# NVIDIA/tacotron2

Measured on AMD Instinct MI355X. Metric: mel-frames/sec (train fwd+bwd) LJSpeech hparams, higher is better.
Workload: dtype bf16; 1 GPU; BASELINE configs[1]: LJSpeech default hparams, batch_size=64/GPU, synthetic LJSpeech-shaped batches, full train step (fwd+loss+bwd+clip+Adam); global_batch=64, parallelism=dp1, optimizer=FusedAdam, compute=bf16 MFMA operands, f32 accumulate/state/master weights

## Files before the change

include/tacotron2_amd.h:

```cpp
#ifndef TACOTRON2_AMD_H
#define TACOTRON2_AMD_H

#include <stdint.h>

#ifdef __cplusplus
extern "C" {
#endif

#define T2AMD_ABI_VERSION 1
#define T2AMD_OK 0
#define T2AMD_ERR_ARG 1
#define T2AMD_ERR_LAUNCH 2

#define T2AMD_ATT_DIM 128
#define T2AMD_LOC_FILTERS 32
#define T2AMD_LOC_KERNEL 31
#define T2AMD_LOC_TAPS (2 * T2AMD_LOC_KERNEL)
#define T2AMD_ATT_SLICES 4

int t2amd_abi_version(void);
const char* t2amd_source_sha1(void);
const char* t2amd_last_error(void);
int t2amd_struct_sizes(int* out, int max_n);
int t2amd_set_validate_only(int on);
// ... 31 lines not shown
                            long long n, int accumulate, int perm_taps, int perm_ci, void* stream);
int t2amd_splitk_reduce2d_f32(const float* partials, int nsplit, long long stride, float* out, int rows, int cols,
                              long long ldo, int accumulate, void* stream);

typedef struct t2amd_gemm16_desc {
    const void* A;
    const void* B;
    float* C;
    int M, N, K;
    long long lda, ldb, ldc;
    int splitk;
    long long strideSplitC;
    int accumulate;
    const float* bias;
    int win_T, win_Tp;
} t2amd_gemm16_desc;
int t2amd_gemm16_tn(const t2amd_gemm16_desc* d, void* stream);
int t2amd_gemm16_kk(const t2amd_gemm16_desc* d, void* stream);
int t2amd_gemm16_kk_group(const t2amd_gemm16_desc* d, int count, void* stream);

int t2amd_cast_halo_bf16(const float* src, long long lds, void* dst, long long rows, int C, int T, int pad, void* stream);

int t2amd_pack_conv_bf16(const float* W, void* out, int Co, int Ci, int k, int Kp, int reversed, void* stream);

int t2amd_transpose_cast_bf16(const void* src, int src_is_bf16, long long lds, void* dst, long long ldd, int rows, int cols,
                              int rows_padded, void* stream);

int t2amd_bn_stats_f32(const float* x, long long ldx, int M, int N, double* ws, float* mean,
                       float* invstd, float* running_mean, float* running_var, float momentum,
                       float eps, void* stream);
int t2amd_bn_eval_invstd_f32(const float* running_var, float* invstd, int N, float eps, void* stream);
// ... 564 lines not shown
```

tacotron2_amd/csrc/gemm16.hip:

```cpp
#include "common.h"
#include <stdlib.h>

typedef __bf16 g16_bf16x8 __attribute__((ext_vector_type(8)));
typedef __attribute__((address_space(3))) void* g16_lptr;
typedef __attribute__((address_space(1))) const void* g16_gptr;

#define G16_T 256
#define G16_BK 64
#define G16_IMG (G16_T * 128)
#define G16_NT 512

struct Gemm16Params {
    t2amd_gemm16_desc d;
    int ktiles_per_split;
};

struct G16Tile { int bx, by, bz; };
__device__ __forceinline__ G16Tile g16_tile_id() {
    const int nbx = gridDim.x, nby = gridDim.y;
    const int total = nbx * nby * (int)gridDim.z;
    const int L = blockIdx.x + nbx * (blockIdx.y + nby * blockIdx.z);
    const int xcd = L & 7, q = L >> 3;
    const int base = total >> 3, rem = total & 7;
    const int id = xcd * base + (xcd < rem ? xcd : rem) + q;
    const int per_z = nbx * nby;
    G16Tile t;
    t.bz = id / per_z;
    const int r = id - t.bz * per_z;
    const int G = 8;
    const int group = r / (G * nbx);
    const int first = group * G;
    const int gsz = (nby - first) < G ? (nby - first) : G;
    const int w = r - group * (G * nbx);
    t.by = first + w % gsz;
    t.bx = w / gsz;
    return t;
}

__global__ __launch_bounds__(G16_NT) void gemm16_tn_kernel(Gemm16Params p) {
    __shared__ __attribute__((aligned(16))) char smem[4 * G16_IMG];
    const t2amd_gemm16_desc& d = p.d;
    const int tid = threadIdx.x, lane = tid & 63;
    const int wave = __builtin_amdgcn_readfirstlane(tid >> 6);
    const int wm = wave >> 2, wn = wave & 3;
    const int l31 = lane & 31, lhi = lane >> 5;

    const G16Tile tile = g16_tile_id();
    const int split = tile.bz;
    const int row0 = tile.by * G16_T, col0 = tile.bx * G16_T;
    const int M = d.M, N = d.N;
    const int nkt_all = d.K / G16_BK;
    const int kt_beg = split * p.ktiles_per_split;
    int kt_end = kt_beg + p.ktiles_per_split;
// ... 91 lines not shown
            asm volatile("s_waitcnt vmcnt(0)" ::: "memory");
            __builtin_amdgcn_s_barrier();
            if (kt + 2 < nk) G16_ISSUE(0)
            G16_TILE(1)
            asm volatile("s_waitcnt vmcnt(0)" ::: "memory");
            __builtin_amdgcn_s_barrier();
        }
        if (nk & 1) G16_TILE(0)
    }
#undef G16_ISSUE
#undef G16_READ
#undef G16_WAIT
#undef G16_MFMA
#undef G16_TILE

    float* __restrict__ C = d.C + (long long)split * d.strideSplitC;
#pragma unroll
    for (int tm = 0; tm < 4; ++tm) {
#pragma unroll
        for (int tn = 0; tn < 2; ++tn) {
            const int gn = col0 + wn * 64 + tn * 32 + l31;
#pragma unroll
            for (int r = 0; r < 16; ++r) {
                const int gm = row0 + wm * 128 + tm * 32 + (r & 3) + 8 * (r >> 2) + 4 * lhi;
                long long crow = gm;
                bool live = gm < M;
                if (d.win_Tp > 0) {
                    const int b_ = gm / d.win_Tp, t_ = gm - b_ * d.win_Tp;
                    live = live && t_ < d.win_T;
                    crow = (long long)b_ * d.win_T + t_;
                }
                if (live && gn < N) {
                    float* cp = C + crow * d.ldc + gn;
                    float val = acc[tm][tn][r];
                    if (d.bias) val += d.bias[gn];
                    if (d.accumulate) val += *cp;
                    *cp = val;
                }
            }
        }
    }
}

extern "C" int t2amd_gemm16_tn(const t2amd_gemm16_desc* dp, void* stream) {
    T2_REQUIRE(dp != nullptr, "gemm16: null descriptor");
    Gemm16Params p;
    p.d = *dp;
    t2amd_gemm16_desc& d = p.d;
    T2_REQUIRE(d.A && d.B && d.C, "gemm16: null operand");
    T2_REQUIRE(d.M > 0 && d.N > 0 && d.K > 0 && d.K % G16_BK == 0, "gemm16: K must be a positive multiple of 64");
    T2_REQUIRE(t2_aligned16(d.A) && t2_aligned16(d.B) && d.lda % 8 == 0 && d.ldb % 8 == 0 && d.ldb >= d.K,
               "gemm16: operands must be 16-byte aligned with row strides that are multiples of 8 elements (B's >= K)");
    T2_REQUIRE(d.win_Tp == 0 || (d.win_T > 0 && d.win_T <= d.win_Tp && d.splitk == 1), "gemm16: bad window geometry");
    T2_REQUIRE(d.win_Tp > 0 || d.lda >= d.K, "gemm16: lda must be >= K unless the rows are windows");
    if (d.splitk < 1) d.splitk = 1;
    T2_REQUIRE(d.splitk == 1 || (!d.bias && !d.accumulate), "gemm16: split-K needs a plain epilogue");
    const int nkt = d.K / G16_BK;
    p.ktiles_per_split = t2_cdiv(nkt, d.splitk);
    dim3 grid(t2_cdiv(d.N, G16_T), t2_cdiv(d.M, G16_T), d.splitk);
    T2_REQUIRE(grid.y <= 65535 && grid.z <= 65535, "gemm16: grid too large");
    T2_LAUNCH(gemm16_tn_kernel, grid, dim3(G16_NT), 0, (hipStream_t)stream, p);
    T2_LAUNCH_CHECK();
    return T2AMD_OK;
}

typedef float g16_f32x2 __attribute__((ext_vector_type(2)));

#define G16_GROUP 4
struct Gemm16GroupParams {
    t2amd_gemm16_desc d[G16_GROUP];
    int coltile_end[G16_GROUP];
    int count;
};

__global__ __launch_bounds__(G16_NT) void gemm16_kk_kernel(Gemm16GroupParams p) {
    __shared__ __attribute__((aligned(16))) char smem[4 * G16_IMG];
    const int tid = threadIdx.x, lane = tid & 63;
    const int wave = __builtin_amdgcn_readfirstlane(tid >> 6);
    const int wm = wave >> 2, wn = wave & 3;
    const int l31 = lane & 31, lhi = lane >> 5;

    const G16Tile tile = g16_tile_id();
    const int split = tile.bz;
    int prob = 0;
#pragma unroll
    for (int j = 0; j + 1 < G16_GROUP; ++j)
        if (j + 1 < p.count && tile.bx >= p.coltile_end[j]) prob = j + 1;
    const int bx = tile.bx - (prob > 0 ? p.coltile_end[prob - 1] : 0);
    struct { const void* A; const void* B; float* C; int M, N, K; long long lda, ldb, ldc; long long strideSplitC; int accumulate;
// ... 127 lines not shown
            KK_LANDED(1, kt + 1)
            if (kt + 2 < nk) KK_ISSUE(0, kt + 2)
            KK_TILE(1)
            KK_LANDED(0, kt + 2)
        }
        if (nk & 1) KK_TILE(0)
    }
#undef KK_ISSUE
#undef KK_LANDED
#undef KK_READ
#undef KK_WAIT
#undef KK_OP
#undef KK_MFMA
#undef KK_TILE

    float* __restrict__ C = d.C + (long long)split * d.strideSplitC;
#pragma unroll
    for (int tm = 0; tm < 4; ++tm) {
#pragma unroll
        for (int tn = 0; tn < 2; ++tn) {
            const int gn = col0 + wn * 64 + tn * 32 + l31;
#pragma unroll
            for (int r = 0; r < 16; ++r) {
                const int gm = row0 + wm * 128 + tm * 32 + (r & 3) + 8 * (r >> 2) + 4 * lhi;
                if (gm < M && gn < N) {
                    float* cp = C + (long long)gm * d.ldc + gn;
                    float val = acc[tm][tn][r];
                    if (d.bias) val += d.bias[gn];
                    if (d.accumulate) val += *cp;
                    *cp = val;
// ... 6 lines not shown
extern "C" int t2amd_gemm16_kk_group(const t2amd_gemm16_desc* dp, int count, void* stream) {
    T2_REQUIRE(dp != nullptr && count >= 1 && count <= G16_GROUP, "gemm16_kk: 1..4 descriptors");
    Gemm16GroupParams p;
    p.count = count;
    int coltiles = 0;
    for (int j = 0; j < G16_GROUP; ++j) {
        p.d[j] = dp[j < count ? j : count - 1];
        if (j >= count) { p.coltile_end[j] = coltiles; continue; }
        t2amd_gemm16_desc& d = p.d[j];
        T2_REQUIRE(d.A && d.B && d.C, "gemm16_kk: null operand");
        T2_REQUIRE(d.M >= 8 && d.N >= 8 && d.K > 0 && d.M % 8 == 0 && d.N % 8 == 0, "gemm16_kk: M and N must be positive multiples of 8, K positive");
        T2_REQUIRE(t2_aligned16(d.A) && t2_aligned16(d.B) && d.lda > 0 && d.ldb > 0 && d.lda % 8 == 0 && d.ldb % 8 == 0,
                   "gemm16_kk: operands must be 16-byte aligned with row strides that are multiples of 8 elements");
        T2_REQUIRE(d.win_Tp == 0 && d.win_T == 0, "gemm16_kk: no window epilogue (overlapping rows are expressed by lda / ldb < M / N)");
        if (d.splitk < 1) d.splitk = 1;
        T2_REQUIRE(d.splitk == 1 || (!d.bias && !d.accumulate), "gemm16_kk: split-K needs a plain epilogue");
        T2_REQUIRE(d.M == p.d[0].M && d.splitk == p.d[0].splitk, "gemm16_kk: the products of one launch share M and the split count");
        coltiles += t2_cdiv(d.N, G16_T);
        p.coltile_end[j] = coltiles;
    }
    dim3 grid(coltiles, t2_cdiv(p.d[0].M, G16_T), p.d[0].splitk);
    T2_REQUIRE(grid.y <= 65535 && grid.z <= 65535, "gemm16_kk: grid too large");
    T2_LAUNCH(gemm16_kk_kernel, grid, dim3(G16_NT), 0, (hipStream_t)stream, p);
    T2_LAUNCH_CHECK();
    return T2AMD_OK;
}

extern "C" int t2amd_gemm16_kk(const t2amd_gemm16_desc* dp, void* stream) { return t2amd_gemm16_kk_group(dp, 1, stream); }

template <bool SRC16>
__global__ __launch_bounds__(256) void transpose_cast16_kernel(const void* __restrict__ src, long long lds_, unsigned short* __restrict__ dst,
                                                               long long ldd, int rows, int cols, int rpad) {
    __shared__ unsigned short tile[64][66];
    const int r0 = blockIdx.x * 64, c0 = blockIdx.y * 64;
    const int tid = threadIdx.x;
    const bool vec_in = SRC16 ? (lds_ % 4 == 0 && (reinterpret_cast<size_t>(src) & 7) == 0) : (lds_ % 4 == 0 && (reinterpret_cast<size_t>(src) & 15) == 0);
#pragma unroll
    for (int pass = 0; pass < 4; ++pass) {
        const int i = pass * 16 + (tid >> 4), j = 4 * (tid & 15);
// ... 113 lines not shown
```

tacotron2_amd/engine.py:

```python
import os

import math
import torch

from . import native as nv
from .native import NativeError

BN_EPS = 1e-5
BN_MOMENTUM = 0.1


def check_hparams(hp):
    if hp.n_frames_per_step != 1:
        raise ValueError("n_frames_per_step != 1 is not supported (nor by the reference, hparams.py:56)")
    K = hp.attention_location_kernel_size
    if not (1 <= hp.attention_dim <= nv.ATT_DIM and 1 <= hp.attention_location_n_filters <= nv.LOC_FILTERS
            and 1 <= K <= nv.LOC_KERNEL and K % 2 == 1):
        raise ValueError("the attention kernels hold attention_dim <= %d, <= %d location filters and an odd location "
                         "kernel <= %d (smaller geometries run zero-embedded in the compiled one; an even kernel size "
                         "does not run in the reference either: ConvNorm pads (k-1)//2, model.py:18-20)"
                         % (nv.ATT_DIM, nv.LOC_FILTERS, nv.LOC_KERNEL))
    for name in ('encoder_embedding_dim', 'attention_rnn_dim', 'decoder_rnn_dim', 'prenet_dim'):
        if getattr(hp, name) % 64 != 0:
            raise ValueError("%s must be a multiple of 64 for the MFMA recurrent kernels" % name)
# ... 73 lines not shown
            best, best_t = s, t
    return best


WGRAD16 = os.environ.get('T2AMD_WGRAD16', '1') != '0'


WGRAD_KK = os.environ.get('T2AMD_WGRAD_KK', '1') != '0'


def _kk_to(run, out, A16, B16, K, M, N, lda=None, ldb=None, perm=None):
    sk = _choose_splitk16(M, N, K)
    if sk == 1 and perm is None:
        nv.gemm16_kk(out, A16, B16, K, M=M, N=N, lda=lda, ldb=ldb)
        return
    part = run.empty(sk, M * N)
    nv.gemm16_kk(part[0].view(M, N), A16, B16, K, M=M, N=N, lda=lda, ldb=ldb, splitk=sk, partials=part)
    if perm is not None:
        nv.splitk_reduce(part, sk, out, perm_taps=perm[0], perm_ci=perm[1])
    else:
        nv.splitk_reduce2d(part, sk, out)


def _lstm_wgrad_kk(run, dG2, B, parts, outs):
    rowsD, G4 = dG2.shape
    widths = [src.shape[1] for src, _ in parts]
    offs = [0]
    for w in widths:
        offs.append(offs[-1] + w)
    jobs = []
    for dW, i0, i1 in outs:
        base = offs[i0]
        for i in range(i0, i1):
            src, shifted = parts[i]
            if src.dtype != torch.bfloat16:
                src = run.cast16(src)
            blk = dW[:, offs[i] - base:offs[i + 1] - base]
            if shifted and rowsD <= B:
                blk.zero_()
            elif shifted:
                jobs.append((blk, dG2[B:], src, rowsD - B, widths[i]))
            else:
                jobs.append((blk, dG2, src, rowsD, widths[i]))
    if not jobs:
        return
    sk = _choose_splitk16(G4, sum((j[4] + 255) // 256 * 256 for j in jobs), rowsD)
    if sk == 1:
        nv.gemm16_kk_group([dict(Cm=blk, A16=A, B16=Bm, K=K, M=G4, N=w) for blk, A, Bm, K, w in jobs])
        return
    parts_ = [run.empty(sk, G4 * w) for _, _, _, _, w in jobs]
    nv.gemm16_kk_group([dict(Cm=pt[0].view(G4, w), A16=A, B16=Bm, K=K, M=G4, N=w, splitk=sk, partials=pt)
                        for (blk, A, Bm, K, w), pt in zip(jobs, parts_)])
    for (blk, _, _, _, _), pt in zip(jobs, parts_):
        nv.splitk_reduce2d(pt, sk, blk)


def _lstm_wgrad16(run, dG2, B, parts, outs):
    rowsD, G4 = dG2.shape
    if WGRAD_KK and G4 % 8 == 0 and all(src.shape[1] % 8 == 0 for src, _ in parts):
        return _lstm_wgrad_kk(run, dG2, B, parts, outs)
    Kp = ((rowsD + B + 63) // 64) * 64
    GT = run.empty16(G4, Kp)
    nv.transpose_cast_bf16(dG2, GT)
    widths = [src.shape[1] for src, _ in parts]
    XT = run.empty16(sum(widths), Kp)
    n0, offs = 0, []
    for (src, shifted), w in zip(parts, widths):
        blk = XT[n0:n0 + w]
        if shifted:
# ... 2 lines not shown
                nv.transpose_cast_bf16(src[:rowsD - B], blk[:, B:])
            else:
                blk[:, B:].zero_()
        else:
            nv.transpose_cast_bf16(src, blk)
        offs.append(n0)
        n0 += w
    offs.append(n0)
    for dW, i0, i1 in outs:
        Bop = XT[offs[i0]:offs[i1]]
        M, N = dW.shape
        sk = _choose_splitk16(M, N, Kp)
        if sk == 1:
            nv.gemm16_tn(dW, GT, Bop)
        else:
            part = run.empty(sk, M * N)
            nv.gemm16_tn(dW, GT, Bop, splitk=sk, partials=part)
            nv.splitk_reduce(part, sk, dW)


class _Ctx(object):
    arena = None

    def release(self):
        a, self.arena = self.arena, None
        _arena_release(a)

    def __del__(self):
        try:
            self.release()
        except Exception:
            pass

# ... 1701 lines not shown
```

tacotron2_amd/native.py:

```python
import ctypes as C
import os

import torch

_HERE = os.path.dirname(os.path.abspath(__file__))
LIB_PATH = os.environ.get("T2AMD_LIB", os.path.join(_HERE, "lib", "libtacotron2_amd.so"))

TORCH_OPS_PATH = os.path.join(_HERE, "lib", "libtacotron2_amd_torch.so")

ATT_DIM = 128
LOC_FILTERS = 32
LOC_KERNEL = 31
LOC_TAPS = 62
ATT_SLICES = 4

_f32p = C.c_void_p
_i64 = C.c_longlong


class GemmDesc(C.Structure):
    _fields_ = [
        ("A", _f32p), ("B", _f32p), ("C", _f32p),
        ("M", C.c_int), ("N", C.c_int), ("K", C.c_int),
        ("lda", _i64), ("ldb", _i64), ("ldc", _i64),
# ... 5 lines not shown
        ("bias", _f32p), ("act", C.c_int),
        ("keep", C.c_void_p), ("ldkeep", _i64), ("keep_scale", C.c_float),
        ("convA_T", C.c_int), ("convA_C", C.c_int), ("convA_pad", C.c_int), ("convA_sign", C.c_int),
        ("convB_T", C.c_int), ("convB_C", C.c_int), ("convB_pad", C.c_int),
        ("precision", C.c_int),
    ]


class Gemm16Desc(C.Structure):
    _fields_ = [
        ("A", C.c_void_p), ("B", C.c_void_p), ("C", _f32p),
        ("M", C.c_int), ("N", C.c_int), ("K", C.c_int),
        ("lda", _i64), ("ldb", _i64), ("ldc", _i64),
        ("splitk", C.c_int), ("strideSplitC", _i64), ("accumulate", C.c_int), ("bias", _f32p),
        ("win_T", C.c_int), ("win_Tp", C.c_int),
    ]


class Seg(C.Structure):
    _fields_ = [("p", _f32p), ("ld", _i64), ("width", C.c_int)]


class LstmStep(C.Structure):
    _fields_ = [
        ("x", Seg * 3), ("nseg", C.c_int),
        ("W", _f32p), ("Ktot", C.c_int), ("H", C.c_int), ("B", C.c_int),
        ("gin", _f32p), ("ld_gin", _i64),
        ("bias", _f32p),
        ("c_prev", _f32p), ("ld_cprev", _i64),
        ("gates_out", _f32p), ("ld_gates", _i64),
# ... 178 lines not shown
    _fields_ = [("param", C.c_void_p * MAX_TENSORS), ("grad", C.c_void_p * MAX_TENSORS),
                ("exp_avg", C.c_void_p * MAX_TENSORS), ("exp_avg_sq", C.c_void_p * MAX_TENSORS),
                ("numel", C.c_longlong * MAX_TENSORS), ("first_block", C.c_int * MAX_TENSORS), ("count", C.c_int)]


class AdamHyper(C.Structure):
    _fields_ = [("step_size", C.c_float), ("bc2_sqrt", C.c_float), ("one_minus_beta1", C.c_float),
                ("beta2", C.c_float), ("one_minus_beta2", C.c_float), ("eps", C.c_float), ("weight_decay", C.c_float)]


_STRUCTS = [GemmDesc, Seg, LstmStep, SkinnyGemm, Addend, LstmBwd, AttnFwd, AttnBwd, DecTrain,
            DecTrainBwd, LstmSeq, DecInfer, SmallLinear, TensorList, AdamHyper, DecPersist, Gemm16Desc]

SYMBOLS = [
    "t2amd_abi_version", "t2amd_source_sha1", "t2amd_last_error", "t2amd_struct_sizes", "t2amd_set_validate_only", "t2amd_profile_enable", "t2amd_profile_read", "t2amd_profile_event_overhead",
    "t2amd_gemm_f32", "t2amd_gemm_tile_size", "t2amd_splitk_reduce_f32", "t2amd_splitk_reduce2d_f32", "t2amd_gemm16_tn", "t2amd_gemm16_kk", "t2amd_gemm16_kk_group", "t2amd_transpose_cast_bf16", "t2amd_cast_halo_bf16", "t2amd_pack_conv_bf16",
    "t2amd_bn_stats_f32", "t2amd_bn_eval_invstd_f32", "t2amd_bn_act_fwd_f32", "t2amd_bn_act_bwd_f32", "t2amd_bn_act_bwd_img_f32", "t2amd_colsum_bf16", "t2amd_bn_act_fwd_img_f32",
    "t2amd_colsum_f32",
    "t2amd_embedding_fwd_f32", "t2amd_embedding_bwd_f32", "t2amd_philox_keep_mask", "t2amd_fill_f32",
    "t2amd_copy2d_f32", "t2amd_cast_bf16_f32", "t2amd_split_bf16x3_f32", "t2amd_transpose_f32", "t2amd_frames_to_time_major_f32",
    "t2amd_split_projection_f32", "t2amd_finalize_outputs_f32", "t2amd_grads_to_channel_last_f32",
    "t2amd_gather_dout_f32", "t2amd_relu_dropout_bwd_f32",
    "t2amd_lstm_step_fwd_f32", "t2amd_skinny_gemm_f32", "t2amd_lstm_pointwise_bwd_f32",
    "t2amd_lstm_step_fwd2_f32", "t2amd_skinny_gemm2_f32", "t2amd_lstm_pointwise_bwd2_f32",
    "t2amd_fold_location_f32", "t2amd_unfold_location_grads_f32",
    "t2amd_attention_step_fwd_f32", "t2amd_attention_step_bwd_f32",
    "t2amd_decoder_train_fwd_loop_f32", "t2amd_decoder_train_bwd_loop_f32",
    "t2amd_decoder_train_fwd_persistent_flag_bytes", "t2amd_decoder_train_fwd_persistent_supported", "t2amd_decoder_train_fwd_persistent_f32",
    "t2amd_lstm_seq_fwd_f32", "t2amd_lstm_seq_bwd_f32", "t2amd_decoder_infer_steps_f32",
    "t2amd_set_decoder_streams", "t2amd_set_bptt_cell_fold", "t2amd_get_bptt_cell_fold", "t2amd_attn_bwd_ws_floats",
    "t2amd_set_small_batch_max", "t2amd_get_small_batch_max", "t2amd_dec_infer_uses_tiles",
# ... 16 lines not shown
]

_P, _I, _L, _F, _UL = C.c_void_p, C.c_int, C.c_longlong, C.c_float, C.c_ulonglong


def _argtypes():
    pt = C.POINTER
    return {
        "t2amd_gemm_f32": [pt(GemmDesc), _P],
        "t2amd_gemm_tile_size": [_I, _I, _I, _I, _I, _I],
        "t2amd_splitk_reduce_f32": [_P, _I, _L, _P, _L, _I, _I, _I, _P],
        "t2amd_splitk_reduce2d_f32": [_P, _I, _L, _P, _I, _I, _L, _I, _P],
        "t2amd_gemm16_tn": [pt(Gemm16Desc), _P],
        "t2amd_gemm16_kk": [pt(Gemm16Desc), _P],
        "t2amd_gemm16_kk_group": [pt(Gemm16Desc), _I, _P],
        "t2amd_transpose_cast_bf16": [_P, _I, _L, _P, _L, _I, _I, _I, _P],
        "t2amd_cast_halo_bf16": [_P, _L, _P, _L, _I, _I, _I, _P],
        "t2amd_pack_conv_bf16": [_P, _P, _I, _I, _I, _I, _I, _P],
        "t2amd_bn_stats_f32": [_P, _L, _I, _I, _P, _P, _P, _P, _P, _F, _F, _P],
        "t2amd_bn_eval_invstd_f32": [_P, _P, _I, _F, _P],
        "t2amd_bn_act_fwd_f32": [_P, _L, _P, _L, _I, _I, _P, _P, _P, _P, _I, _P, _L, _F, _P, _I, _P],
        "t2amd_bn_act_fwd_img_f32": [_P, _L, _P, _L, _I, _I, _P, _P, _P, _P, _I, _P, _L, _F, _P, _I, _I, _P],
        "t2amd_bn_act_bwd_f32": [_P, _L, _P, _L, _P, _L, _I, _I, _P, _P, _P, _I, _P, _L, _F, _P, _P, _P, _P],
        "t2amd_bn_act_bwd_img_f32": [_P, _L, _P, _L, _P, _L, _I, _I, _P, _P, _P, _I, _P, _L, _F, _P, _P, _P, _P, _I, _I, _P, _I, _P],
        "t2amd_colsum_f32": [_P, _L, _I, _I, _P, _P, _I, _P],
        "t2amd_colsum_bf16": [_P, _L, _I, _I, _P, _P, _I, _P],
        "t2amd_embedding_fwd_f32": [_P, _P, _P, _L, _I, _I, _P],
        "t2amd_embedding_bwd_f32": [_P, _P, _P, _P, _L, _I, _I, _P],
        "t2amd_philox_keep_mask": [_P, _L, _F, _UL, _UL, _P],
        "t2amd_fill_f32": [_P, _L, _F, _P],
# ... 118 lines not shown
    lib = C.CDLL(LIB_PATH)
    for name in SYMBOLS:
        if not hasattr(lib, name):
            raise NativeError("tacotron2_amd: symbol %s missing from %s" % (name, LIB_PATH))
    for name, at in _argtypes().items():
        fn = getattr(lib, name)
        fn.argtypes = at
        fn.restype = C.c_int
    lib.t2amd_last_error.restype = C.c_char_p
    lib.t2amd_reflect_index.argtypes = [_L, _L]
    lib.t2amd_reflect_index.restype = C.c_longlong
    lib.t2amd_gl_packed_rows.argtypes = [_P, _I, _I, _I]
    lib.t2amd_gl_packed_rows.restype = C.c_longlong
    lib.t2amd_abi_version.restype = C.c_int
    lib.t2amd_attn_bwd_ws_floats.restype = C.c_longlong
    lib.t2amd_attn_fwd_ws_floats.restype = C.c_longlong
    lib.t2amd_decoder_persist_mailbox_bytes.restype = C.c_longlong
    lib.t2amd_lstm_seq_persistent_mailbox_bytes.restype = C.c_longlong
    lib.t2amd_lstm_seq_batch_persistent_flag_bytes.restype = C.c_longlong
    lib.t2amd_decoder_train_fwd_persistent_flag_bytes.restype = C.c_longlong
    if lib.t2amd_abi_version() != 1:
        raise NativeError("tacotron2_amd: ABI version mismatch")
    lib.t2amd_source_sha1.restype = C.c_char_p
    lib.t2amd_source_sha1.argtypes = []
    built = (lib.t2amd_source_sha1() or b"").decode()
    if os.path.isdir(os.path.join(_HERE, "csrc")) and os.environ.get("T2AMD_ALLOW_STALE_LIB", "0") != "1":
        from . import build as _build
        try:
            want = _build.source_sha1()
        except OSError as e:
# ... 232 lines not shown
            raise NativeError("gemm: keep mask must be a [M,N] uint8 view, got %s" % (tuple(keep.shape),))
        d.keep, d.ldkeep, d.keep_scale = ptr(keep, torch.uint8), keep.stride(0), keep_scale
    if convA is not None:
        d.convA_T, d.convA_C, d.convA_pad, d.convA_sign = convA
    if convB is not None:
        d.convB_T, d.convB_C, d.convB_pad = convB
    if splitk > 1:
        if partials is None or partials.numel() < splitk * M * N or not partials.is_contiguous():
            raise NativeError("gemm: split-K needs a contiguous partials buffer")
        d.C = ptr(partials)
        d.ldc = N
        d.strideSplitC = M * N
    _check(lib.t2amd_gemm_f32(C.byref(d), _stream()), "t2amd_gemm_f32")


def gemm16_tn(Cm, A16, B16, K=None, splitk=1, partials=None, accumulate=False, bias=None):
    lib = load()
    d = Gemm16Desc()
    pa, lda, M, Ka = _mat(A16, torch.bfloat16)
    pb, ldb, N, Kb = _mat(B16, torch.bfloat16)
    K = Ka if K is None else K
    if K > Ka or K > Kb or Cm.shape[0] != M or Cm.shape[1] != N:
        raise NativeError("gemm16_tn: shape mismatch A=%s B=%s C=%s K=%d" % (tuple(A16.shape), tuple(B16.shape), tuple(Cm.shape), K))
    d.A, d.B, d.M, d.N, d.K, d.lda, d.ldb = pa, pb, M, N, K, lda, ldb
    d.splitk = splitk
    if splitk > 1:
        if partials is None or partials.numel() < splitk * M * N:
            raise NativeError("gemm16_tn: split-K needs a (splitk, M*N) partials buffer")
        d.C, d.ldc, d.strideSplitC = ptr(partials), N, M * N
    else:
        d.C, d.ldc = _mat(Cm)[:2]
    d.accumulate = 1 if accumulate else 0
    d.bias = ptr(bias)
    _check(lib.t2amd_gemm16_tn(C.byref(d), _stream()), "t2amd_gemm16_tn")


def conv16(Cm, img16, W16, B, T, pad, bias=None, accumulate=False):
    lib = load()
    d = Gemm16Desc()
    Ci = img16.shape[1]
    Tp = T + 2 * pad
    pw, ldw, Co, K = _mat(W16, torch.bfloat16)
    klen = (2 * pad + 1) * Ci
    if img16.shape[0] < B * Tp + 2 * pad or K < klen or K - klen > 2 * pad * Ci or Cm.shape[0] != B * T or Cm.shape[1] != Co:
        raise NativeError("conv16: shape mismatch img=%s W=%s C=%s" % (tuple(img16.shape), tuple(W16.shape), tuple(Cm.shape)))
    d.A, d.lda = ptr(_fullc(img16), torch.bfloat16), Ci
    d.B, d.ldb = pw, ldw
    d.C, d.ldc = _mat(Cm)[:2]
    d.M, d.N, d.K = (B - 1) * Tp + T, Co, K
    d.splitk, d.accumulate, d.bias = 1, 1 if accumulate else 0, ptr(bias)
    d.win_T, d.win_Tp = T, Tp
    _check(lib.t2amd_gemm16_tn(C.byref(d), _stream()), "t2amd_gemm16_tn")


def _kk_desc(Cm, A16, B16, K, M=None, N=None, lda=None, ldb=None, splitk=1, partials=None, accumulate=False, bias=None):
    d = Gemm16Desc()
    pa, lda0, ra, wa = _mat(A16, torch.bfloat16)
    pb, ldb0, rb, wb = _mat(B16, torch.bfloat16)
    M = wa if M is None else M
    N = wb if N is None else N
    lda = lda0 if lda is None else lda
    ldb = ldb0 if ldb is None else ldb
    span_a = (ra - 1) * lda0 + wa
    span_b = (rb - 1) * ldb0 + wb
    if K < 1 or (K - 1) * lda + M > span_a or (K - 1) * ldb + N > span_b or Cm.shape[0] != M or Cm.shape[1] != N:
        raise NativeError("gemm16_kk: shape mismatch A=%s B=%s C=%s M=%d N=%d K=%d lda=%d ldb=%d"
                          % (tuple(A16.shape), tuple(B16.shape), tuple(Cm.shape), M, N, K, lda, ldb))
    d.A, d.B, d.M, d.N, d.K, d.lda, d.ldb = pa, pb, M, N, K, lda, ldb
    d.splitk = splitk
    if splitk > 1:
        if partials is None or partials.numel() < splitk * M * N:
            raise NativeError("gemm16_kk: split-K needs a (splitk, M*N) partials buffer")
        d.C, d.ldc, d.strideSplitC = ptr(partials), N, M * N
    else:
        d.C, d.ldc = _mat(Cm)[:2]
    d.accumulate = 1 if accumulate else 0
    d.bias = ptr(bias)
    return d


def gemm16_kk(Cm, A16, B16, K, M=None, N=None, lda=None, ldb=None, splitk=1, partials=None, accumulate=False, bias=None):
    d = _kk_desc(Cm, A16, B16, K, M, N, lda, ldb, splitk, partials, accumulate, bias)
    _check(load().t2amd_gemm16_kk(C.byref(d), _stream()), "t2amd_gemm16_kk")


def gemm16_kk_group(problems):
    if not 1 <= len(problems) <= 4:
        raise NativeError("gemm16_kk_group: 1..4 problems, got %d" % len(problems))
    arr = (Gemm16Desc * len(problems))(*[_kk_desc(**kw) for kw in problems])
    reads = [kw[k_] for kw in problems for k_ in ('A16', 'B16')]
    writes = [kw['partials'] if kw.get('partials') is not None else kw['Cm'] for kw in problems]
    if not _via_ops("wgrad_gemm16", [arr], reads, writes):
        _check(load().t2amd_gemm16_kk_group(arr, len(problems), _stream()), "t2amd_gemm16_kk_group")


def pack_conv_bf16(W, reversed=False):
    Co, Ci, k = W.shape
    rows, inner = (Ci, Co) if reversed else (Co, Ci)
    Kp = (k * inner + 63) // 64 * 64
    out = torch.empty(rows, Kp, dtype=torch.bfloat16, device=W.device)
    _check(load().t2amd_pack_conv_bf16(ptr(_fullc(W)), ptr(out, torch.bfloat16), Co, Ci, k, Kp, 1 if reversed else 0, _stream()),
           "t2amd_pack_conv_bf16")
    return out


def cast_halo_bf16(src, dst, T, pad):
# ... 1187 lines not shown
```

Measured before the change: 648,400 valid mel-frames/s.

## Fuse split-K reduction into gemm16 kernels via per-tile arrival counters

Split-K bf16 GEMMs now write per-tile partials to a workspace, and the last-arriving CTA per output tile (found through an atomic counter) sums all splits and writes the final result, with optional tap/channel permutation and accumulation. This removes the separate splitk_reduce launches and the large M*N slab round trip when the grid has enough tiles and the workspace fits. It adds atomics, cache-bypassing loads and stores, a serial reduction done by one CTA per tile, and shared counters that must return to zero, which is unsafe if kernels on different streams overlap.

```diff
diff --git a/include/tacotron2_amd.h b/include/tacotron2_amd.h
--- a/include/tacotron2_amd.h
+++ b/include/tacotron2_amd.h
@@ -69,7 +69,13 @@
     int accumulate;
     const float* bias;
     int win_T, win_Tp;
+    float* ws;
+    int* counters;
+    int perm_taps, perm_ci;
 } t2amd_gemm16_desc;
+int t2amd_set_gemm16_fused_splitk(int mode);
+int t2amd_get_gemm16_fused_splitk(void);
+long long t2amd_gemm16_splitk_ws_floats(int M, int N, int splitk);
 int t2amd_gemm16_tn(const t2amd_gemm16_desc* d, void* stream);
 int t2amd_gemm16_kk(const t2amd_gemm16_desc* d, void* stream);
 int t2amd_gemm16_kk_group(const t2amd_gemm16_desc* d, int count, void* stream);
diff --git a/tacotron2_amd/csrc/gemm16.hip b/tacotron2_amd/csrc/gemm16.hip
--- a/tacotron2_amd/csrc/gemm16.hip
+++ b/tacotron2_amd/csrc/gemm16.hip
@@ -37,6 +37,98 @@
     return t;
 }
 
+
+#define G16_TILE_FLOATS (G16_T * G16_T)
+static __device__ __forceinline__ void g16_store_sc1(float* p, f32x4 v) {
+    asm volatile("global_store_dwordx4 %0, %1, off sc1" : : "v"(p), "v"(v) : "memory");
+}
+#define G16_LOAD_SC1(V_, P_) asm volatile("global_load_dwordx4 %0, %1, off sc1" : "=&v"(V_) : "v"(P_) : "memory")
+
+struct G16FusedOut {
+    float* C; long long ldc; int M, N, splitk, accumulate, perm_taps, perm_ci;
+    float* ws; int* counters;
+};
+
+static __device__ __forceinline__ void g16_fused_epilogue(char* smem, const f32x16 (&acc)[4][2], const G16FusedOut& o, int tile_index,
+                                                          int split, int row0, int col0) {
+    const int tid = threadIdx.x, lane = tid & 63;
+    const int wave = __builtin_amdgcn_readfirstlane(tid >> 6);
+    const int wm = wave >> 2, wn = wave & 3;
+    const int l31 = lane & 31, lhi = lane >> 5;
+    const int sk = o.splitk;
+    float* const tile_ws = o.ws + (long long)tile_index * sk * G16_TILE_FLOATS;
+    const int lane_off = wave * (8 * 4 * 256) + lane * 4;
+    {
+        float* mine = tile_ws + (long long)split * G16_TILE_FLOATS + lane_off;
+#pragma unroll
+        for (int tm = 0; tm < 4; ++tm)
+#pragma unroll
+            for (int tn = 0; tn < 2; ++tn) {
+                if (row0 + wm * 128 + tm * 32 >= o.M || col0 + wn * 64 + tn * 32 >= o.N) continue;
+#pragma unroll
+                for (int q = 0; q < 4; ++q)
+                    g16_store_sc1(mine + ((tm * 2 + tn) * 4 + q) * 256,
+                                  f32x4{acc[tm][tn][4 * q], acc[tm][tn][4 * q + 1], acc[tm][tn][4 * q + 2], acc[tm][tn][4 * q + 3]});
+            }
+    }
+    asm volatile("s_waitcnt vmcnt(0)" ::: "memory");
+    __syncthreads();
+    if (tid == 0)
+        *reinterpret_cast<int*>(smem) = __hip_atomic_fetch_add(o.counters + tile_index, 1, __ATOMIC_RELAXED, __HIP_MEMORY_SCOPE_AGENT);
+    __syncthreads();
+    if (*reinterpret_cast<volatile int*>(smem) != sk - 1) return;
+
+    const float* first = tile_ws + lane_off;
+#pragma unroll 1
+    for (int t = 0; t < 8; ++t) {
+        const int tm = t >> 1, tn = t & 1;
+        if (row0 + wm * 128 + tm * 32 >= o.M || col0 + wn * 64 + tn * 32 >= o.N) continue;
+        f32x4 s[4];
+#pragma unroll
+        for (int q = 0; q < 4; ++q) s[q] = f32x4{0.f, 0.f, 0.f, 0.f};
+        const float* src = first + t * (4 * 256);
+#pragma unroll 1
+        for (int k = 0; k < sk; k += 4) {
+            f32x4 v[4][4];
+#pragma unroll
+            for (int j = 0; j < 4; ++j) {
+                const float* sp = src + (long long)(k + j < sk ? k + j : sk - 1) * G16_TILE_FLOATS;
+#pragma unroll
+                for (int q = 0; q < 4; ++q) G16_LOAD_SC1(v[j][q], sp + q * 256);
+            }
+            asm volatile("s_waitcnt vmcnt(0)"
+                         : "+v"(v[0][0]), "+v"(v[0][1]), "+v"(v[0][2]), "+v"(v[0][3]), "+v"(v[1][0]), "+v"(v[1][1]), "+v"(v[1][2]),
+                           "+v"(v[1][3]), "+v"(v[2][0]), "+v"(v[2][1]), "+v"(v[2][2]), "+v"(v[2][3]), "+v"(v[3][0]), "+v"(v[3][1]),
+                           "+v"(v[3][2]), "+v"(v[3][3]) : : "memory");
+#pragma unroll
+            for (int j = 0; j < 4; ++j)
+                if (k + j < sk) {
+#pragma unroll
+                    for (int q = 0; q < 4; ++q) s[q] += v[j][q];
+                }
+        }
+        const int gn = col0 + wn * 64 + tn * 32 + l31;
+        if (gn >= o.N) continue;
+#pragma unroll
+        for (int q = 0; q < 4; ++q)
+#pragma unroll
+            for (int e = 0; e < 4; ++e) {
+                const int gm = row0 + wm * 128 + tm * 32 + e + 8 * q + 4 * lhi;
+                if (gm >= o.M) continue;
+                long long idx = (long long)gm * o.ldc + gn;
+                if (o.perm_taps > 0) {
+                    const int tap = gn / o.perm_ci, ci = gn - tap * o.perm_ci;
+                    idx = (long long)gm * o.N + (long long)ci * o.perm_taps + tap;
+                }
+                float val = s[q][e];
+                if (o.accumulate) val += o.C[idx];
+                o.C[idx] = val;
+            }
+    }
+    if (tid == 0) __hip_atomic_store(o.counters + tile_index, 0, __ATOMIC_RELAXED, __HIP_MEMORY_SCOPE_AGENT);
+}
+
+template <bool FUSED>
 __global__ __launch_bounds__(G16_NT) void gemm16_tn_kernel(Gemm16Params p) {
     __shared__ __attribute__((aligned(16))) char smem[4 * G16_IMG];
     const t2amd_gemm16_desc& d = p.d;
@@ -158,6 +250,13 @@
 #undef G16_MFMA
 #undef G16_TILE
 
+    if (FUSED) {
+        G16FusedOut o;
+        o.C = d.C; o.ldc = d.ldc; o.M = M; o.N = N; o.splitk = d.splitk; o.accumulate = d.accumulate;
+        o.perm_taps = d.perm_taps; o.perm_ci = d.perm_ci; o.ws = d.ws; o.counters = d.counters;
+        g16_fused_epilogue(smem, acc, o, tile.by * (int)gridDim.x + tile.bx, split, row0, col0);
+        return;
+    }
     float* __restrict__ C = d.C + (long long)split * d.strideSplitC;
 #pragma unroll
     for (int tm = 0; tm < 4; ++tm) {
@@ -186,6 +285,43 @@
     }
 }
 
+static int g_fused_splitk = -1;
+static int g16_fused_mode() {
+    if (g_fused_splitk < 0) {
+        const char* e = getenv("T2AMD_GEMM16_FUSED_SPLITK");
+        g_fused_splitk = e && e[0] >= '0' && e[0] <= '2' && !e[1] ? e[0] - '0' : 1;
+    }
+    return g_fused_splitk;
+}
+extern "C" int t2amd_set_gemm16_fused_splitk(int mode) {
+    T2_REQUIRE(mode >= 0 && mode <= 2, "set_gemm16_fused_splitk: 0 (slabs + reduce launch), 1 (in the launch where it pays), 2 (always in the launch)");
+    g_fused_splitk = mode;
+    return T2AMD_OK;
+}
+extern "C" int t2amd_get_gemm16_fused_splitk(void) { return g16_fused_mode(); }
+extern "C" long long t2amd_gemm16_splitk_ws_floats(int M, int N, int splitk) {
+    if (M <= 0 || N <= 0 || splitk <= 0) return 0;
+    return (long long)splitk * t2_cdiv(M, G16_T) * t2_cdiv(N, G16_T) * G16_TILE_FLOATS;
+}
+static bool g16_use_fused(int splitk, long long tiles) {
+    const int mode = g16_fused_mode();
+    if (mode != 1) return mode == 2;
+    return tiles >= 64 && (long long)splitk * tiles * (G16_TILE_FLOATS * 4) <= (256ll << 20);
+}
+static bool g16_check_managed(const t2amd_gemm16_desc& d) {
+    if (!d.counters || !t2_aligned16(d.ws) || d.ldc < d.N) return false;
+    if (d.perm_taps < 0 || (d.perm_taps > 0 && (d.perm_ci <= 0 || (long long)d.perm_taps * d.perm_ci != d.N || d.ldc != d.N))) return false;
+    return true;
+}
+static void g16_to_slabs(t2amd_gemm16_desc& d) {
+    d.C = d.ws; d.ldc = d.N; d.strideSplitC = (long long)d.M * d.N; d.accumulate = 0;
+}
+static int g16_reduce_slabs(const t2amd_gemm16_desc& d, void* stream) {
+    const long long mn = (long long)d.M * d.N;
+    if (d.ldc == d.N) return t2amd_splitk_reduce_f32(d.ws, d.splitk, mn, d.C, mn, d.accumulate, d.perm_taps, d.perm_ci, stream);
+    return t2amd_splitk_reduce2d_f32(d.ws, d.splitk, mn, d.C, d.M, d.N, d.ldc, d.accumulate, stream);
+}
+
 extern "C" int t2amd_gemm16_tn(const t2amd_gemm16_desc* dp, void* stream) {
     T2_REQUIRE(dp != nullptr, "gemm16: null descriptor");
     Gemm16Params p;
@@ -198,14 +334,24 @@
     T2_REQUIRE(d.win_Tp == 0 || (d.win_T > 0 && d.win_T <= d.win_Tp && d.splitk == 1), "gemm16: bad window geometry");
     T2_REQUIRE(d.win_Tp > 0 || d.lda >= d.K, "gemm16: lda must be >= K unless the rows are windows");
     if (d.splitk < 1) d.splitk = 1;
-    T2_REQUIRE(d.splitk == 1 || (!d.bias && !d.accumulate), "gemm16: split-K needs a plain epilogue");
+    const bool managed = d.splitk > 1 && d.ws != nullptr;
+    T2_REQUIRE(d.splitk == 1 || !d.bias, "gemm16: split-K takes no bias");
+    T2_REQUIRE(managed || d.splitk == 1 || !d.accumulate, "gemm16: split-K into caller-reduced slabs needs a plain epilogue");
+    if (managed) T2_REQUIRE(g16_check_managed(d), "gemm16: bad split-K workspace (16-byte aligned ws, counters, perm_taps * perm_ci == N == ldc)");
     const int nkt = d.K / G16_BK;
     p.ktiles_per_split = t2_cdiv(nkt, d.splitk);
     dim3 grid(t2_cdiv(d.N, G16_T), t2_cdiv(d.M, G16_T), d.splitk);
     T2_REQUIRE(grid.y <= 65535 && grid.z <= 65535, "gemm16: grid too large");
-    T2_LAUNCH(gemm16_tn_kernel, grid, dim3(G16_NT), 0, (hipStream_t)stream, p);
+    if (managed && g16_use_fused(d.splitk, (long long)grid.x * grid.y)) {
+        T2_LAUNCH((gemm16_tn_kernel<true>), grid, dim3(G16_NT), 0, (hipStream_t)stream, p);
+        T2_LAUNCH_CHECK();
+        return T2AMD_OK;
+    }
+    const t2amd_gemm16_desc final_ = d;
+    if (managed) g16_to_slabs(d);
+    T2_LAUNCH((gemm16_tn_kernel<false>), grid, dim3(G16_NT), 0, (hipStream_t)stream, p);
     T2_LAUNCH_CHECK();
-    return T2AMD_OK;
+    return managed ? g16_reduce_slabs(final_, stream) : T2AMD_OK;
 }
 
 typedef float g16_f32x2 __attribute__((ext_vector_type(2)));
@@ -217,6 +363,7 @@
     int count;
 };
 
+template <bool FUSED>
 __global__ __launch_bounds__(G16_NT) void gemm16_kk_kernel(Gemm16GroupParams p) {
     __shared__ __attribute__((aligned(16))) char smem[4 * G16_IMG];
     const int tid = threadIdx.x, lane = tid & 63;
@@ -374,6 +521,14 @@
 #undef KK_MFMA
 #undef KK_TILE
 
+    if (FUSED) {
+        G16FusedOut o;
+        o.C = d.C; o.ldc = d.ldc; o.M = M; o.N = N; o.splitk = d.splitk; o.accumulate = d.accumulate;
+        o.perm_taps = p.d[prob].perm_taps; o.perm_ci = p.d[prob].perm_ci; o.ws = p.d[prob].ws; o.counters = p.d[prob].counters;
+        const int nbx = (prob > 0 ? p.coltile_end[prob] - p.coltile_end[prob - 1] : p.coltile_end[0]);
+        g16_fused_epilogue(smem, acc, o, tile.by * nbx + bx, split, row0, col0);
+        return;
+    }
     float* __restrict__ C = d.C + (long long)split * d.strideSplitC;
 #pragma unroll
     for (int tm = 0; tm < 4; ++tm) {
@@ -410,15 +565,36 @@
                    "gemm16_kk: operands must be 16-byte aligned with row strides that are multiples of 8 elements");
         T2_REQUIRE(d.win_Tp == 0 && d.win_T == 0, "gemm16_kk: no window epilogue (overlapping rows are expressed by lda / ldb < M / N)");
         if (d.splitk < 1) d.splitk = 1;
-        T2_REQUIRE(d.splitk == 1 || (!d.bias && !d.accumulate), "gemm16_kk: split-K needs a plain epilogue");
-        T2_REQUIRE(d.M == p.d[0].M && d.splitk == p.d[0].splitk, "gemm16_kk: the products of one launch share M and the split count");
+        const bool managed_j = d.splitk > 1 && d.ws != nullptr;
+        T2_REQUIRE(d.splitk == 1 || !d.bias, "gemm16_kk: split-K takes no bias");
+        T2_REQUIRE(managed_j || d.splitk == 1 || !d.accumulate, "gemm16_kk: split-K into caller-reduced slabs needs a plain epilogue");
+        if (managed_j) T2_REQUIRE(g16_check_managed(d), "gemm16_kk: bad split-K workspace (16-byte aligned ws, counters, perm_taps * perm_ci == N == ldc)");
+        T2_REQUIRE(d.M == p.d[0].M && d.splitk == p.d[0].splitk && (d.ws != nullptr) == (p.d[0].ws != nullptr),
+                   "gemm16_kk: the products of one launch share M, the split count and who reduces");
         coltiles += t2_cdiv(d.N, G16_T);
         p.coltile_end[j] = coltiles;
     }
     dim3 grid(coltiles, t2_cdiv(p.d[0].M, G16_T), p.d[0].splitk);
     T2_REQUIRE(grid.y <= 65535 && grid.z <= 65535, "gemm16_kk: grid too large");
-    T2_LAUNCH(gemm16_kk_kernel, grid, dim3(G16_NT), 0, (hipStream_t)stream, p);
+    const bool managed = p.d[0].splitk > 1 && p.d[0].ws != nullptr;
+    if (managed && g16_use_fused(p.d[0].splitk, (long long)grid.x * grid.y)) {
+        T2_LAUNCH((gemm16_kk_kernel<true>), grid, dim3(G16_NT), 0, (hipStream_t)stream, p);
+        T2_LAUNCH_CHECK();
+        return T2AMD_OK;
+    }
+    t2amd_gemm16_desc final_[G16_GROUP];
+    for (int j = 0; j < count; ++j) {
+        final_[j] = p.d[j];
+        if (managed) g16_to_slabs(p.d[j]);
+    }
+    for (int j = count; j < G16_GROUP; ++j) p.d[j] = p.d[count - 1];
+    T2_LAUNCH((gemm16_kk_kernel<false>), grid, dim3(G16_NT), 0, (hipStream_t)stream, p);
     T2_LAUNCH_CHECK();
+    if (managed)
+        for (int j = 0; j < count; ++j) {
+            const int rc = g16_reduce_slabs(final_[j], stream);
+            if (rc != T2AMD_OK) return rc;
+        }
     return T2AMD_OK;
 }
 
diff --git a/tacotron2_amd/engine.py b/tacotron2_amd/engine.py
--- a/tacotron2_amd/engine.py
+++ b/tacotron2_amd/engine.py
@@ -111,12 +111,13 @@
     if sk == 1 and perm is None:
         nv.gemm16_kk(out, A16, B16, K, M=M, N=N, lda=lda, ldb=ldb)
         return
-    part = run.empty(sk, M * N)
-    nv.gemm16_kk(part[0].view(M, N), A16, B16, K, M=M, N=N, lda=lda, ldb=ldb, splitk=sk, partials=part)
-    if perm is not None:
-        nv.splitk_reduce(part, sk, out, perm_taps=perm[0], perm_ci=perm[1])
-    else:
-        nv.splitk_reduce2d(part, sk, out)
+    if sk > 1:
+        nv.gemm16_kk(out if perm is None else out.view(M, N), A16, B16, K, M=M, N=N, lda=lda, ldb=ldb, splitk=sk,
+                     ws=run.empty(nv.gemm16_splitk_ws_floats(M, N, sk)), perm=perm)
+        return
+    part = run.empty(1, M * N)
+    nv.gemm16_kk(part[0].view(M, N), A16, B16, K, M=M, N=N, lda=lda, ldb=ldb)
+    nv.splitk_reduce(part, 1, out, perm_taps=perm[0], perm_ci=perm[1])
 
 
 def _lstm_wgrad_kk(run, dG2, B, parts, outs):
@@ -145,11 +146,8 @@
     if sk == 1:
         nv.gemm16_kk_group([dict(Cm=blk, A16=A, B16=Bm, K=K, M=G4, N=w) for blk, A, Bm, K, w in jobs])
         return
-    parts_ = [run.empty(sk, G4 * w) for _, _, _, _, w in jobs]
-    nv.gemm16_kk_group([dict(Cm=pt[0].view(G4, w), A16=A, B16=Bm, K=K, M=G4, N=w, splitk=sk, partials=pt)
-                        for (blk, A, Bm, K, w), pt in zip(jobs, parts_)])
-    for (blk, _, _, _, _), pt in zip(jobs, parts_):
-        nv.splitk_reduce2d(pt, sk, blk)
+    nv.gemm16_kk_group([dict(Cm=blk, A16=A, B16=Bm, K=K, M=G4, N=w, splitk=sk, ws=run.empty(nv.gemm16_splitk_ws_floats(G4, w, sk)))
+                        for blk, A, Bm, K, w in jobs])
 
 
 def _lstm_wgrad16(run, dG2, B, parts, outs):
@@ -182,9 +180,7 @@
         if sk == 1:
             nv.gemm16_tn(dW, GT, Bop)
         else:
-            part = run.empty(sk, M * N)
-            nv.gemm16_tn(dW, GT, Bop, splitk=sk, partials=part)
-            nv.splitk_reduce(part, sk, dW)
+            nv.gemm16_tn(dW, GT, Bop, splitk=sk, ws=run.empty(nv.gemm16_splitk_ws_floats(M, N, sk)))
 
 
 class _Ctx(object):
diff --git a/tacotron2_amd/native.py b/tacotron2_amd/native.py
--- a/tacotron2_amd/native.py
+++ b/tacotron2_amd/native.py
@@ -43,6 +43,7 @@
         ("lda", _i64), ("ldb", _i64), ("ldc", _i64),
         ("splitk", C.c_int), ("strideSplitC", _i64), ("accumulate", C.c_int), ("bias", _f32p),
         ("win_T", C.c_int), ("win_Tp", C.c_int),
+        ("ws", _f32p), ("counters", C.c_void_p), ("perm_taps", C.c_int), ("perm_ci", C.c_int),
     ]
 
 
@@ -251,7 +252,7 @@
 
 SYMBOLS = [
     "t2amd_abi_version", "t2amd_source_sha1", "t2amd_last_error", "t2amd_struct_sizes", "t2amd_set_validate_only", "t2amd_profile_enable", "t2amd_profile_read", "t2amd_profile_event_overhead",
-    "t2amd_gemm_f32", "t2amd_gemm_tile_size", "t2amd_splitk_reduce_f32", "t2amd_splitk_reduce2d_f32", "t2amd_gemm16_tn", "t2amd_gemm16_kk", "t2amd_gemm16_kk_group", "t2amd_transpose_cast_bf16", "t2amd_cast_halo_bf16", "t2amd_pack_conv_bf16",
+    "t2amd_gemm_f32", "t2amd_gemm_tile_size", "t2amd_splitk_reduce_f32", "t2amd_splitk_reduce2d_f32", "t2amd_gemm16_tn", "t2amd_gemm16_kk", "t2amd_gemm16_kk_group", "t2amd_set_gemm16_fused_splitk", "t2amd_get_gemm16_fused_splitk", "t2amd_gemm16_splitk_ws_floats", "t2amd_transpose_cast_bf16", "t2amd_cast_halo_bf16", "t2amd_pack_conv_bf16",
     "t2amd_bn_stats_f32", "t2amd_bn_eval_invstd_f32", "t2amd_bn_act_fwd_f32", "t2amd_bn_act_bwd_f32", "t2amd_bn_act_bwd_img_f32", "t2amd_colsum_bf16", "t2amd_bn_act_fwd_img_f32",
     "t2amd_colsum_f32",
     "t2amd_embedding_fwd_f32", "t2amd_embedding_bwd_f32", "t2amd_philox_keep_mask", "t2amd_fill_f32",
@@ -298,6 +299,9 @@
         "t2amd_gemm16_tn": [pt(Gemm16Desc), _P],
         "t2amd_gemm16_kk": [pt(Gemm16Desc), _P],
         "t2amd_gemm16_kk_group": [pt(Gemm16Desc), _I, _P],
+        "t2amd_set_gemm16_fused_splitk": [_I],
+        "t2amd_get_gemm16_fused_splitk": [],
+        "t2amd_gemm16_splitk_ws_floats": [_I, _I, _I],
         "t2amd_transpose_cast_bf16": [_P, _I, _L, _P, _L, _I, _I, _I, _P],
         "t2amd_cast_halo_bf16": [_P, _L, _P, _L, _I, _I, _I, _P],
         "t2amd_pack_conv_bf16": [_P, _P, _I, _I, _I, _I, _I, _P],
@@ -446,6 +450,7 @@
     lib.t2amd_gl_packed_rows.restype = C.c_longlong
     lib.t2amd_abi_version.restype = C.c_int
     lib.t2amd_attn_bwd_ws_floats.restype = C.c_longlong
+    lib.t2amd_gemm16_splitk_ws_floats.restype = C.c_longlong
     lib.t2amd_attn_fwd_ws_floats.restype = C.c_longlong
     lib.t2amd_decoder_persist_mailbox_bytes.restype = C.c_longlong
     lib.t2amd_lstm_seq_persistent_mailbox_bytes.restype = C.c_longlong
@@ -708,7 +713,48 @@
     _check(lib.t2amd_gemm_f32(C.byref(d), _stream()), "t2amd_gemm_f32")
 
 
-def gemm16_tn(Cm, A16, B16, K=None, splitk=1, partials=None, accumulate=False, bias=None):
+GEMM16_MAX_TILES = 4096
+_g16_counters = {}
+
+
+def set_gemm16_fused_splitk(mode):
+    _check(load().t2amd_set_gemm16_fused_splitk(int(mode)), "t2amd_set_gemm16_fused_splitk")
+
+
+def get_gemm16_fused_splitk():
+    return load().t2amd_get_gemm16_fused_splitk()
+
+
+def gemm16_splitk_ws_floats(M, N, splitk):
+    return int(load().t2amd_gemm16_splitk_ws_floats(M, N, splitk))
+
+
+def gemm16_counters(device=None):
+    if _validate_only:
+        return torch.zeros(GEMM16_MAX_TILES, dtype=torch.int32)
+    key = (torch.cuda.current_device(), torch.cuda.current_stream().cuda_stream)
+    c = _g16_counters.get(key)
+    if c is None:
+        c = _g16_counters[key] = torch.zeros(GEMM16_MAX_TILES, dtype=torch.int32, device='cuda')
+    return c
+
+
+def _g16_managed(d, name, Cm, M, N, splitk, ws, counters, perm, first_tile=0):
+    tiles = ((M + 255) // 256) * ((N + 255) // 256)
+    if ws.dtype != torch.float32 or not ws.is_contiguous() or ws.numel() < gemm16_splitk_ws_floats(M, N, splitk):
+        raise NativeError("%s: split-K workspace needs gemm16_splitk_ws_floats(M, N, splitk) contiguous floats" % name)
+    counters = gemm16_counters() if counters is None else counters
+    if counters.dtype != torch.int32 or not counters.is_contiguous() or first_tile + tiles > counters.numel():
+        raise NativeError("%s: %d output tiles need as many int32 arrival counters" % (name, first_tile + tiles))
+    d.C, d.ldc = _mat(Cm)[:2]
+    d.ws = ptr(ws)
+    d.counters = (counters.data_ptr() + 4 * first_tile) if (counters.is_cuda or _validate_only) else None
+    if perm is not None:
+        d.perm_taps, d.perm_ci = perm
+    return tiles
+
+
+def gemm16_tn(Cm, A16, B16, K=None, splitk=1, partials=None, accumulate=False, bias=None, ws=None, counters=None, perm=None):
     lib = load()
     d = Gemm16Desc()
     pa, lda, M, Ka = _mat(A16, torch.bfloat16)
@@ -718,7 +764,9 @@
         raise NativeError("gemm16_tn: shape mismatch A=%s B=%s C=%s K=%d" % (tuple(A16.shape), tuple(B16.shape), tuple(Cm.shape), K))
     d.A, d.B, d.M, d.N, d.K, d.lda, d.ldb = pa, pb, M, N, K, lda, ldb
     d.splitk = splitk
-    if splitk > 1:
+    if splitk > 1 and ws is not None:
+        _g16_managed(d, "gemm16_tn", Cm, M, N, splitk, ws, counters, perm)
+    elif splitk > 1:
         if partials is None or partials.numel() < splitk * M * N:
             raise NativeError("gemm16_tn: split-K needs a (splitk, M*N) partials buffer")
         d.C, d.ldc, d.strideSplitC = ptr(partials), N, M * N
@@ -747,7 +795,8 @@
     _check(lib.t2amd_gemm16_tn(C.byref(d), _stream()), "t2amd_gemm16_tn")
 
 
-def _kk_desc(Cm, A16, B16, K, M=None, N=None, lda=None, ldb=None, splitk=1, partials=None, accumulate=False, bias=None):
+def _kk_desc(Cm, A16, B16, K, M=None, N=None, lda=None, ldb=None, splitk=1, partials=None, accumulate=False, bias=None,
+             ws=None, counters=None, perm=None, first_tile=0):
     d = Gemm16Desc()
     pa, lda0, ra, wa = _mat(A16, torch.bfloat16)
     pb, ldb0, rb, wb = _mat(B16, torch.bfloat16)
@@ -762,7 +811,9 @@
                           % (tuple(A16.shape), tuple(B16.shape), tuple(Cm.shape), M, N, K, lda, ldb))
     d.A, d.B, d.M, d.N, d.K, d.lda, d.ldb = pa, pb, M, N, K, lda, ldb
     d.splitk = splitk
-    if splitk > 1:
+    if splitk > 1 and ws is not None:
+        _g16_managed(d, "gemm16_kk", Cm, M, N, splitk, ws, counters, perm, first_tile)
+    elif splitk > 1:
         if partials is None or partials.numel() < splitk * M * N:
             raise NativeError("gemm16_kk: split-K needs a (splitk, M*N) partials buffer")
         d.C, d.ldc, d.strideSplitC = ptr(partials), N, M * N
@@ -773,17 +824,24 @@
     return d
 
 
-def gemm16_kk(Cm, A16, B16, K, M=None, N=None, lda=None, ldb=None, splitk=1, partials=None, accumulate=False, bias=None):
-    d = _kk_desc(Cm, A16, B16, K, M, N, lda, ldb, splitk, partials, accumulate, bias)
+def gemm16_kk(Cm, A16, B16, K, M=None, N=None, lda=None, ldb=None, splitk=1, partials=None, accumulate=False, bias=None,
+              ws=None, counters=None, perm=None):
+    d = _kk_desc(Cm, A16, B16, K, M, N, lda, ldb, splitk, partials, accumulate, bias, ws, counters, perm)
     _check(load().t2amd_gemm16_kk(C.byref(d), _stream()), "t2amd_gemm16_kk")
 
 
 def gemm16_kk_group(problems):
     if not 1 <= len(problems) <= 4:
         raise NativeError("gemm16_kk_group: 1..4 problems, got %d" % len(problems))
-    arr = (Gemm16Desc * len(problems))(*[_kk_desc(**kw) for kw in problems])
+    descs, first = [], 0
+    for kw in problems:
+        descs.append(_kk_desc(first_tile=first, **kw))
+        if kw.get('ws') is not None and kw.get('splitk', 1) > 1:
+            first += ((descs[-1].M + 255) // 256) * ((descs[-1].N + 255) // 256)
+    arr = (Gemm16Desc * len(problems))(*descs)
     reads = [kw[k_] for kw in problems for k_ in ('A16', 'B16')]
     writes = [kw['partials'] if kw.get('partials') is not None else kw['Cm'] for kw in problems]
+    writes += [kw['ws'] for kw in problems if kw.get('ws') is not None]
     if not _via_ops("wgrad_gemm16", [arr], reads, writes):
         _check(load().t2amd_gemm16_kk_group(arr, len(problems), _stream()), "t2amd_gemm16_kk_group")
 
```

Result: no change. 647,600 valid mel-frames/s (median of 3 runs) (-0.1%).
